# etemesi254/zune-jpeg

Hardware: NVIDIA B200
Metric: decoded MP/s (dequant+IDCT+upsample+YCbCr→RGB), 4K 4:2:0 batch @1/2/4/8 B200 (higher is better)
Workload: dtype int32

## Files before the change

### zune-jpeg_b200/csrc/zj_capi.cu

```cuda
#include <cuda_runtime.h>
#include <stdint.h>
#include <stdio.h>
#include <stdlib.h>
#include <string.h>

#include <algorithm>
#include <atomic>
#include <chrono>
#include <functional>
#include <mutex>
#include <new>
#include <thread>
#include <vector>

#include "../../include/zune_jpeg_b200.h"
#include "zj_device.h"

namespace zj {
cudaError_t launch_group(const DevImage *d_images, const LaunchGroup &g, cudaStream_t stream);
cudaError_t launch_convert(const ConvImage *d_images, uint32_t count, uint32_t nc, uint32_t max_ow, uint32_t max_oh, const zj_output_desc &d, cudaStream_t s);
cudaError_t launch_resize(const ResizeImage *d_images, uint32_t count, uint32_t nc, const zj_output_desc &d, const zj_resize &r, cudaStream_t s);
}

using namespace zj;
// ... 96 lines not shown
    d.mcu_x = mcu_x; d.n_strips = n_strips;
    d.Wp = img->comp[0].width_stride;
    d.W = img->n_comp == 3 ? img->comp[1].width_stride : 0;
    d.stride = w * (uint32_t)nc;
    d.T = 0xffffffffu;
    d.small_width = 0;
    d.hv_avx = (mode == MODE_HV && img->variant == ZJ_VARIANT_X86 && (size_t)16 * d.W >= 500) ? 1u : 0u;
    for (uint32_t z = 0; z < img->n_comp; z++)
        for (int k = 0; k < 32; k++)
            d.qtw[z][k] = (uint32_t)img->comp[z].qt[2 * k] | ((uint32_t)img->comp[z].qt[2 * k + 1] << 24);

    if (kind == OUT_GRAY) {
        const size_t len = (size_t)rows * d.Wp;
        if (n_strips > 0 && len / w != rows) return ZJ_ERR_REF_PANIC;
        d.gray_rows_ok = 1;
        d.gray_brows = n_strips * (rows / 8);
        pl->fast = img->variant == ZJ_VARIANT_X86 && !getenv("ZJ_NO_FAST");
        if (pl->fast) {
            const uint32_t ucols = (d.Wp + 15) / 16;
            d.n_tiles = (ucols + ZF_XU_GRAY - 1) / ZF_XU_GRAY;
            d.tile_q = ucols / d.n_tiles;
            d.tile_r = ucols % d.n_tiles;
            pl->grid_strips = (d.gray_brows + 1) / 2;
        } else {
            d.n_tiles = (d.Wp / 8 + ZJ_THREADS - 1) / ZJ_THREADS;
        }
        pl->grid_tiles = d.n_tiles;
    } else if (kind == OUT_YCC) {
        d.n_norm = w; d.P = 3 * w;
    } else if (kind == OUT_RGB) {
        if (w < 16) {
            if (d.Wp > 16) return ZJ_ERR_REF_PANIC;
            d.small_width = 1;
        } else {
            const uint32_t E = d.Wp / 16 > 0 ? d.Wp / 16 - 1 : 0;
            d.n_norm = 16 * E;
            d.P = 48 * E;
            if (d.P > d.stride) return ZJ_ERR_REF_PANIC;
            const uint32_t room = d.stride - d.P;
            const uint32_t diff = room < 64 ? 64 - room : 0;
            d.T = d.P > diff ? d.P - diff : 0;
            if (d.T + 48 > d.stride) return ZJ_ERR_REF_PANIC;
        }
    }
    if (kind != OUT_GRAY) {
        pl->fast = img->variant == ZJ_VARIANT_X86 && (kind == OUT_RGB || kind == OUT_YCC) && !d.small_width && (d.stride & 3u) == 0 &&
                   (mode != MODE_HV || d.hv_avx) && (reinterpret_cast<uintptr_t>(out) & 3) == 0 && !getenv("ZJ_NO_FAST");
        if (pl->fast) {
            const uint32_t xuv[4] = {ZF_XU_NONE, ZF_XU_H, ZF_XU_V, ZF_XU_HV};
            const uint32_t ucols = (d.Wp + 15) / 16;
            d.n_tiles = (ucols + xuv[mode] - 1) / xuv[mode];
            d.tile_q = ucols / d.n_tiles;
            d.tile_r = ucols % d.n_tiles;
        } else {
            const int tmv[4] = {TM_NONE, TM_H, TM_V, TM_HV};
            d.n_tiles = (mcu_x + tmv[mode] - 1) / tmv[mode];
            d.tile_q = mcu_x / d.n_tiles;
            d.tile_r = mcu_x % d.n_tiles;
        }
        pl->grid_tiles = d.n_tiles;
        d.magic_w = d.W ? (((uint64_t)1 << 40) + d.W - 1) / d.W : 0;
    }
    return ZJ_OK;
}

static int check_buffers(const zj_image *img, const Plan &pl, const void *out, size_t out_len)
{
    for (uint32_t z = 0; z < pl.ncomp_used; z++) {
        if (!img->comp[z].coeff) return ZJ_ERR_INVALID_ARG;
        if (img->comp[z].n_i16 < (uint64_t)pl.n_strips * pl.chunk[z]) return ZJ_ERR_SHORT_PLANE;
    }
    if (!out) return ZJ_ERR_INVALID_ARG;
    if (out_len < pl.out_size) return ZJ_ERR_SHORT_OUTPUT;
    return ZJ_OK;
}

static int check_device_alignment(const zj_image *img, const Plan &pl)
{
    for (uint32_t z = 0; z < pl.ncomp_used; z++)
        if (reinterpret_cast<uintptr_t>(img->comp[z].coeff) & 15) return ZJ_ERR_INVALID_ARG;
    return ZJ_OK;
}

struct zj_batch {
    int device;
    std::vector<LaunchGroup> groups;
    std::vector<std::pair<uint8_t *, size_t>> zero_only;
    DevImage *d_images;
    size_t n_images;
    uint64_t algo_bytes;
    cudaStream_t pool_stream;
    bool pooled;
};

static cudaMemPool_t g_pool[64] = {};
static std::mutex g_pool_mu;
static cudaMemPool_t device_pool(int device)
{
    if (device < 0 || device >= 64) return nullptr;
    std::lock_guard<std::mutex> lock(g_pool_mu);
    if (!g_pool[device]) {
        cudaMemPoolProps props = {};
        props.allocType = cudaMemAllocationTypePinned;
        props.handleTypes = cudaMemHandleTypeNone;
        props.location.type = cudaMemLocationTypeDevice;
        props.location.id = device;
// ... 996 lines not shown
```

### zune-jpeg_b200/csrc/zj_kernels.cu

```cuda
#include <cuda_runtime.h>
#include <stdint.h>
#include <stdlib.h>

#include <type_traits>

#include "zj_device.h"

#define ZF_LIKELY(x) __builtin_expect(!!(x), 1)
#define ZF_UNLIKELY(x) __builtin_expect(!!(x), 0)

namespace zj {

typedef uint32_t u32;

template <int K> __device__ __forceinline__ u32 madk(u32 a, u32 c) { u32 d; asm("mad.lo.s32 %0, %1, %2, %3;" : "=r"(d) : "r"(a), "n"(K), "r"(c)); return d; }

template <int SH>
__device__ __forceinline__ void idct8(u32 &s0, u32 &s1, u32 &s2, u32 &s3, u32 &s4, u32 &s5, u32 &s6, u32 &s7, const u32 bias)
{
    const u32 p1 = (s2 + s6) * 2217u;
    const u32 t2 = madk<-7567>(s6, p1), t3 = madk<3135>(s2, p1);
    const u32 v = (s0 << 12) + bias;
    const u32 t0 = madk<4096>(s4, v), t1 = madk<-4096>(s4, v);
    const u32 x0 = t0 + t3, x3 = t0 - t3, x1 = t1 + t2, x2 = t1 - t2;
// ... 968 lines not shown
    u32 w[12];
#pragma unroll
    for (int k = 0; k < 4; k++) {
        const u32 yE = evens(yw[k]), yO = odds(yw[k]);
        u32 c0E, c1E, c2E, c0O, c1O, c2O;
        if (ycc) {
            c0E = yE; c1E = cbE[k]; c2E = crE[k]; c0O = yO; c1O = cbO[k]; c2O = crO[k];
        } else {
            convert_pair_hi(yE, cbE[k], crE[k], c0E, c1E, c2E, kk, kr);
            convert_pair_hi(yO, cbO[k], crO[k], c0O, c1O, c2O, kk, kr);
        }
        const u32 rgE = prmt(c0E, c1E, sel);
        const u32 brO = prmt(c2E, c0O, sel);
        const u32 gbO = prmt(c1O, c2O, sel);
        w[3 * k] = prmt(rgE, brO, 0x5410u);
        w[3 * k + 1] = prmt(gbO, rgE, 0x7610u);
        w[3 * k + 2] = prmt(brO, gbO, 0x7632u);
    }
    if (ZF_LIKELY(vec && nw == 12)) {
        uint4 *d = reinterpret_cast<uint4 *>(dst);
        d[0] = make_uint4(w[0], w[1], w[2], w[3]); d[1] = make_uint4(w[4], w[5], w[6], w[7]); d[2] = make_uint4(w[8], w[9], w[10], w[11]);
    } else if (vec && nw == 8) {
        uint4 *d = reinterpret_cast<uint4 *>(dst);
        d[0] = make_uint4(w[0], w[1], w[2], w[3]); d[1] = make_uint4(w[4], w[5], w[6], w[7]);
    } else {
        u32 *d = reinterpret_cast<u32 *>(dst);
#pragma unroll
        for (int k = 0; k < 12; k++) if (k < nw) d[k] = w[k];
    }
}

__device__ __forceinline__ void load16(const uint8_t *p, const bool a16, u32 w[4])
{
    if (a16) { const uint4 v = *reinterpret_cast<const uint4 *>(p); w[0] = v.x; w[1] = v.y; w[2] = v.z; w[3] = v.w; }
    else { const uint2 v0 = *reinterpret_cast<const uint2 *>(p), v1 = *reinterpret_cast<const uint2 *>(p + 8); w[0] = v0.x; w[1] = v0.y; w[2] = v1.x; w[3] = v1.y; }
}

constexpr int ZF_NB = 2;
enum { BAR_FULL = 1, BAR_EMPTY = 3, BAR_QUEUE = 5 };

template <int MODE>
__global__ void __launch_bounds__(ZF_THREADS, ZF_MINBLOCKS)
reconstruct_fast_kernel(const DevImage *__restrict__ images, const int spc)
{
    typedef FastTraits<MODE> FT;
    typedef uint8_t ST;
    constexpr int ROWS = FT::ROWS, TWY = FT::TWY, CS = FT::CS, NRG = FT::NRG, XU = FT::XU, RPU = FT::RPU;
    constexpr bool HALO = FT::NSLOT > 0;

    extern __shared__ __align__(128) uint8_t sDynAll[];
    ST *const sPlanes = sDynAll + 3 * ZF_PRODUCERS * 128 + 128;
    __shared__ __align__(16) u32 sQ[3][32];
    __shared__ int sSlowN;
    __shared__ unsigned short sSlow[ZJ_SLOW_CAP];

    const DevImage &im = images[blockIdx.z];
    const u32 tile = blockIdx.x;
    if (tile >= im.n_tiles) return;
    const int tid = threadIdx.x;
    const u32 stride = im.stride;
    uint8_t *__restrict__ out = im.out;
    const u32 n_strips = im.n_strips;
    const u32 s_begin = blockIdx.y * (u32)spc;

    if (s_begin >= n_strips) {
        if (s_begin >= n_strips + (u32)spc) return;
        const size_t lo = (size_t)n_strips * ROWS * stride, hi = (size_t)im.height * stride;
        if (lo >= hi) return;
        const size_t span = hi - lo, per = (span + im.n_tiles - 1) / im.n_tiles;
        size_t b0 = lo + (size_t)tile * per, b1 = b0 + per;
        if (b1 > hi) b1 = hi;
        for (size_t b = b0 + tid; b < b1; b += ZF_THREADS) out[b] = 0;
        return;
    }
    const int n_it = (int)(min(s_begin + (u32)spc, n_strips) - s_begin);

    const int nt = (int)im.n_tiles;
    const int u0 = (int)(tile * im.tile_q + min(tile, im.tile_r)), u1 = (int)((tile + 1) * im.tile_q + min(tile + 1, im.tile_r));
    const int Wp = (int)im.Wp, W = (int)im.W, mcu_x = (int)im.mcu_x;
    const int X0 = 16 * u0;
    const int yb0 = 2 * u0, nyb = min(2 * u1, Wp >> 3) - yb0;
    const int cb0 = FT::H == 2 ? u0 : yb0, ncb = FT::H == 2 ? u1 - u0 : nyb;
    const int lhb = HALO ? (cb0 == 0 ? mcu_x - 1 : cb0 - 1) : -1;
    const int rhb = HALO ? (cb0 + ncb == mcu_x ? 0 : cb0 + ncb) : -1;
    const int spb = (MODE == MODE_HV && tile == 0 && nt > 1) ? mcu_x - 2 : -1;
    const u32 n_norm = im.n_norm, T = im.T, P = im.P;

    for (int k = tid; k < 96; k += ZF_THREADS) sQ[k >> 5][k & 31] = im.qtw[k >> 5][k & 31];
    if (tid == 0) sSlowN = 0;
    __syncthreads();

    const bool producer = tid < ZF_PRODUCERS;
    const int rtid = producer ? tid : tid - ZF_PRODUCERS;
    if (producer) {
        constexpr int NHB = FT::NSLOT * FT::CBR;
        const int lane = tid & 31, wq = ((rtid >> 5) + (int)(blockIdx.x + blockIdx.y + blockIdx.z)) & 3;
        const int ybpr = Wp >> 3;
        auto decode = [&](int b, int &comp, int &br, int &gcol, int &lcol) {
            if (b < FT::NY) { comp = 0; br = b / FT::YB; const int bc = b % FT::YB; gcol = bc < nyb ? yb0 + bc : -1; lcol = bc * 8; }
            else if (b < FT::NY + 2 * FT::NC) {
                int c = b - FT::NY; comp = 1 + c / FT::NC; c %= FT::NC;
                br = c / FT::CB; const int bc = c % FT::CB; gcol = bc < ncb ? cb0 + bc : -1; lcol = 8 + bc * 8;
            } else {
                int hx = b - FT::NY - 2 * FT::NC; comp = 1 + hx / (NHB > 0 ? NHB : 1); hx %= (NHB > 0 ? NHB : 1);
                const int slot = hx / FT::CBR; br = hx % FT::CBR;
                gcol = slot == 0 ? lhb : (slot == 1 ? rhb : spb);
                lcol = slot == 0 ? 0 : (slot == 1 ? 8 + ncb * 8 : 16 + ncb * 8);
                if (NHB == 0 || comp > 2) { comp = 1; gcol = -1; }
            }
        };
        auto block_ptr = [&](int comp, int br, int gcol) -> const int16_t * {
            return comp == 0 ? im.coeff[0] + (((size_t)s_begin * FT::YBR + br) * ybpr + gcol) * 64
                             : im.coeff[comp] + (((size_t)s_begin * FT::CBR + br) * mcu_x + gcol) * 64;
        };
        const u32 stepY = (u32)(FT::YBR * ybpr * 64), stepC = (u32)(FT::CBR * mcu_x * 64);
        auto setup_job = [&](const int B0, u32 &pkj, const int16_t *&g0, const int16_t *&g1, u32 &jmj) {
            int comp, br, gcol, lcol;
            decode(B0 + lane, comp, br, gcol, lcol);
            const bool active = gcol >= 0;
            pkj = (comp == 0 ? (u32)(br * 8 * TWY + lcol) : (u32)(FT::YBYTES + (comp - 1) * FT::CBYTES + br * 8 * CS + lcol)) |
                  (active ? 0x10000u : 0u) | (comp ? 0x20000u : 0u) | ((u32)comp << 18) |
                  ((comp != 0 && lcol == 0) ? 0x100000u : 0u);
            const int lsub = lane >> 3, lch = lane & 7;
            g0 = g1 = im.coeff[0];
            int mode = 0, lim0 = 0, lim1 = 0;
            if (FT::DENSE) {
                if (active) { mode = 3; g0 = block_ptr(comp, br, gcol); }
            } else if (B0 < FT::NY + 2 * FT::NC) {
                int c0, b0r, gg0, l0;
                decode(B0, c0, b0r, gg0, l0);
                const bool isY = B0 < FT::NY;
                const int bpr = isY ? FT::YB : FT::CB;
                const int col0 = isY ? (B0 % FT::YB) : ((B0 - FT::NY) % FT::NC) % FT::CB;
                const int have = (isY ? nyb : ncb) - col0;
                const int first = (isY ? yb0 : cb0) + col0;
                if (bpr >= 32) { mode = 1; lim0 = min(max(have, 0), 32) - lsub; g0 = block_ptr(c0, b0r, first) + lsub * 64 + lch * 8; }
                else {
                    mode = 2; lim0 = lim1 = min(max(have, 0), 16) - lsub;
                    g0 = block_ptr(c0, b0r, first) + lsub * 64 + lch * 8;
                    g1 = block_ptr(c0, b0r + 1, first) + lsub * 64 + lch * 8;
                }
            } else if (active) { mode = 3; g0 = block_ptr(comp, br, gcol); }
            u32 m = 0;
            for (int k = 0; k < 8; k++) {
                const bool second = mode == 2 && k >= 4;
                if ((mode == 1 || mode == 2) && 4 * (second ? k - 4 : k) < (second ? lim1 : lim0)) m |= 1u << k;
            }
            if (mode == 3) m = 0x100u;
            if (mode == 2) g1 -= 4 * 256;
            else g1 = g0;
            jmj = m;
        };
        const u32 stage0 = (u32)__cvta_generic_to_shared(sDynAll) + (u32)(wq * 32) * 128u;
        const u32 d_even = stage0 + (u32)(lane >> 3) * 128u + (u32)(((lane & 7) ^ (lane >> 3)) * 16);
        const u32 d_odd = stage0 + (u32)(lane >> 3) * 128u + (u32)(((lane & 7) ^ ((lane >> 3) + 4)) * 16);
        const u32 slx = (stage0 + (u32)lane * 128u) | (u32)((lane & 7) * 16);
        const u32 scr = (u32)__cvta_generic_to_shared(sDynAll) + ZF_PRODUCERS * 128u + (u32)rtid * 16u;
        const u32 zslot = ((u32)__cvta_generic_to_shared(sDynAll) + 3u * ZF_PRODUCERS * 128u) | (u32)((lane & 7) * 16);
        if (rtid < 8) sts128(zslot - (u32)((lane & 7) * 16) + (u32)rtid * 16u, 0u, 0u, 0u, 0u);
        asm volatile("bar.sync %0, %1;" ::"r"((int)BAR_QUEUE + 1), "n"(ZF_PRODUCERS) : "memory");
        asm volatile("" : "+r"(const_cast<u32 &>(d_even)), "+r"(const_cast<u32 &>(d_odd)), "+r"(const_cast<u32 &>(slx)), "+r"(const_cast<u32 &>(scr)));
        auto issue = [&](const int16_t *g0, const int16_t *g1, const u32 m) {
            if (ZF_LIKELY(m == 0xffu)) {
#pragma unroll
                for (int k = 0; k < 8; k++)
                    asm volatile("cp.async.cg.shared.global [%0], [%1], 16;" ::"r"(((k & 1) ? d_odd : d_even) + k * 512u), "l"((k < 4 ? g0 : g1) + k * 256) : "memory");
            } else if (m & 0x100u) {
#pragma unroll
                for (int r = 0; r < 8; r++)
                    asm volatile("cp.async.cg.shared.global [%0], [%1], 16;" ::"r"(slx ^ (u32)(r << 4)), "l"(g0 + r * 8) : "memory");
            } else {
#pragma unroll
                for (int k = 0; k < 8; k++)
                    if (m & (1u << k))
                        asm volatile("cp.async.cg.shared.global [%0], [%1], 16;" ::"r"(((k & 1) ? d_odd : d_even) + k * 512u), "l"((k < 4 ? g0 : g1) + k * 256) : "memory");
            }
            asm volatile("cp.async.commit_group;" ::: "memory");
        };
        u32 pk[2], jm[2];
        const int16_t *q0[2], *q1[2];
#pragma unroll
        for (int ps = 0; ps < 2; ps++) {
            const int jw = ps == 0 ? wq : ((wq + ((MODE == MODE_NONE || MODE == MODE_H) ? 2 : 0)) & 3);
            setup_job(ps * ZF_PRODUCERS + jw * 32, pk[ps], q0[ps], q1[ps], jm[ps]);
        }
        const int16_t *qa0 = q0[0], *qb0 = q1[0], *qa1 = q0[1], *qb1 = q1[1];
        const u32 pk0 = pk[0], pk1 = pk[1], jm0 = jm[0], jm1 = jm[1];
        const u32 st0 = FT::DENSE ? ((pk0 & 0x20000u) ? stepC : stepY) : ((wq * 32 < FT::NY) ? stepY : stepC);
        const u32 st1 = FT::DENSE ? ((pk1 & 0x20000u) ? stepC : stepY) : ((ZF_PRODUCERS + wq * 32 < FT::NY) ? stepY : stepC);
        const bool work0 = __any_sync(0xffffffffu, (pk0 & 0x10000u) != 0), work1 = __any_sync(0xffffffffu, (pk1 & 0x10000u) != 0);
        issue(qa0, qb0, jm0);
        qa0 += st0; qb0 += st0;
        int buf = 0;
        for (int it = 0; it < n_it; it++) {
            ST *planes = sPlanes + buf * FT::BUF;
#pragma unroll 1
            for (int ps = 0; ps < 2; ps++) {
                if (ps == 1 && !work1) break;
                const u32 pkk = ps ? pk1 : pk0;
                const bool active = (pkk & 0x10000u) != 0;
                asm volatile("cp.async.wait_group 0;" ::: "memory");
                __syncwarp();
                if (ps == 0 && it >= ZF_NB) bar_sync(BAR_EMPTY + buf);
                auto refill = [&]() {
                    const bool nxt = ps || !work1;
                    issue(nxt ? qa0 : qa1, nxt ? qb0 : qb1, nxt ? (it + 1 < n_it ? jm0 : 0u) : jm1);
                    if (nxt) { qa0 += st0; qb0 += st0; } else { qa1 += st1; qb1 += st1; }
                };
                if (ps ? work1 : work0) idct_rolled<FT::IDCT_UNROLL, FT::LO6>(active, active ? slx : zslot, scr, sQ[(pkk >> 18) & 3u], planes + (pkk & 0xffffu), (pkk & 0x20000u) ? CS : TWY, refill);
                else refill();
            }
            bar_arrive(BAR_FULL + buf);
            buf = buf + 1 == ZF_NB ? 0 : buf + 1;
        }
        return;
    }

    const int tc = rtid;
    const int xu = tc % XU, rgA = tc / XU;
    const bool ycc = im.out_kind == OUT_YCC;
    u32 esel = !ycc ? 0x7351u : 0x6240u, ekk = 0xC000C000u ^ ((u32)spc >> 30);
    asm volatile("" : "+r"(esel), "+r"(ekk));
    u32 ekr = 0x98619861u ^ ((u32)spc >> 30);
    asm volatile("" : "+r"(ekr));
    int xs = X0 + 16 * xu;
    int kind = 0;
    int dst_off = 3 * xs, nw = 12;
    if (u0 + xu < u1 && rgA < NRG / 2) {
        if ((u32)(xs + 16) <= n_norm) {
            kind = 1;
            if (T != 0xffffffffu && (u32)(3 * xs + 48) > T && (u32)(3 * xs) < T + 48) {
                const int keep = (int)T - 3 * xs;
                if ((u32)(3 * xs + 48) > T + 48) kind = 2;
                else if (keep <= 0) kind = 0;
                else if ((keep & 3) == 0) nw = keep >> 2;
                else kind = 2;
            }
        } else if (T != 0xffffffffu && (u0 + xu) == ((Wp - 16) >> 4)) {
            kind = 1; xs = Wp - 16; dst_off = (int)T;
        } else if ((u32)xs < n_norm) {
            kind = 2;
        }
    }
    if (kind == 1 && (dst_off & 3) != 0) kind = 2;
    const bool vec = ((stride & 15u) == 0) && ((reinterpret_cast<uintptr_t>(out) & 15) == 0) && ((dst_off & 15) == 0) && ((nw & 3) == 0);
    const int xl = xs - X0;
    const bool y16 = (xl & 15) == 0;
    const int cc0 = FT::H == 2 ? xs >> 1 : xs;
    const int lc = 8 + (cc0 - cb0 * 8);
    const bool first_x = HALO && cc0 == 0, last_x = HALO && cc0 + 8 == W;
    int kindA = kind, kindB = kind;
    int off0 = 0, off2 = 0;
    bool sel0 = false, firstvec = false, hv_tail = false;
    const int pbit = rgA & 1;
    if (MODE == MODE_H) {
        off0 = first_x ? -CS : 0; off2 = last_x ? CS : 0;
    } else if (MODE == MODE_HV) {
        off0 = (first_x && pbit) ? -CS : 0; off2 = last_x ? CS : 0;
        sel0 = (((pbit ? W : 0) + cc0) & 15) == 0;
        firstvec = pbit == 0 && cc0 < 16;
        hv_tail = pbit == 1 && cc0 + 16 >= W;
        if (kind == 1 && hv_tail && W - 36 - cb0 * 8 < (cb0 == 0 ? 0 : -8)) kindA = kindB = 2;
        if (kind == 1 && firstvec && W < 48) kindA = kindB = 2;
    }
#pragma unroll
    for (int h = 0; h < 2; h++)
        if ((h ? kindB : kindA) == 2) {
            const int slot = atomicAdd(&sSlowN, 1);
            if (slot < ZJ_SLOW_CAP) sSlow[slot] = (unsigned short)(((rgA + h * (NRG / 2)) << 8) | (xl >> 3));
        }
    bar_sync_consumers(BAR_QUEUE);
    const int nslow = sSlowN;

    const u32 z0 = (T != 0xffffffffu && T + 48 > P) ? T + 48 : P;
    const u32 zlen = stride > z0 ? stride - z0 : 0;
    const int zg = (((z0 | stride) & 15u) == 0 && (reinterpret_cast<uintptr_t>(out) & 15) == 0) ? 16 : ((((z0 | stride) & 3u) == 0 && (reinterpret_cast<uintptr_t>(out) & 3) == 0) ? 4 : 1);
    const u32 zper = ((zlen / zg + nt - 1) / nt) * zg;
    const u32 zb0 = min(z0 + tile * zper, stride), zb1 = min(zb0 + zper, stride);
    const int zcnt = (int)((zb1 - zb0) / zg);
    const int zrpp = (zcnt > 0 && zcnt < ZF_CONSUMERS) ? ZF_CONSUMERS / zcnt : 1;
    const int zr0 = (zcnt > 0 && zcnt < ZF_CONSUMERS) ? (tc / zcnt < zrpp ? tc / zcnt : ROWS) : 0;
    const int zk0 = (zcnt > 0 && zcnt < ZF_CONSUMERS) ? tc % zcnt : tc;

    int buf = 0;
    for (int it = 0; it < n_it; it++) {
        const ST *planes = sPlanes + buf * FT::BUF;
        const u32 y_base = (s_begin + it) * ROWS;
        bar_sync(BAR_FULL + buf);
#pragma unroll 1
        for (int h = 0; h < 2; h++) {
            if ((h ? kindB : kindA) != 1) continue;
            const int rg = rgA + h * (NRG / 2);
            int yl0, yl1, ra, rb;
            if (MODE == MODE_V) { yl0 = 2 * rg; yl1 = yl0 + 1; ra = rg; rb = (rg == 0 || rg == 7) ? rg : rg + 1; }
            else if (MODE == MODE_HV) { const int j = rg >> 1; yl0 = 4 * j + pbit; yl1 = yl0 + 2; ra = 2 * j + pbit; rb = (j == 0 || j == 7) ? ra : ra + 2; }
            else { yl0 = rg; yl1 = rg; ra = rg; rb = rg; }
            u32 E0[2][4], O0[2][4], E1[2][4], O1[2][4];
#pragma unroll
            for (int c = 0; c < 2; c++) {
                const uint8_t *base = planes + FT::YBYTES + c * FT::CBYTES;
                if (MODE == MODE_NONE) {
                    u32 w[4];
                    load16(base + ra * CS + lc, false, w);
#pragma unroll
                    for (int k = 0; k < 4; k++) { E0[c][k] = evens(w[k]); O0[c][k] = odds(w[k]); }
                } else if (MODE == MODE_V) {
                    u32 a[4], b[4];
                    load16(base + ra * CS + lc, false, a);
                    load16(base + rb * CS + lc, false, b);
#pragma unroll
                    for (int k = 0; k < 4; k++) {
                        const u32 aE = evens(a[k]), aO = odds(a[k]), bE = evens(b[k]), bO = odds(b[k]);
                        T2pair(aE, bE, E0[c][k], E1[c][k]);
                        T2pair(aO, bO, O0[c][k], O1[c][k]);
                    }
                } else if (MODE == MODE_H) {
                    const uint8_t *pa = base + ra * CS + lc;
                    const uint2 a = *reinterpret_cast<const uint2 *>(pa);
                    const bool hstart = first_x && rg == 0, hend = last_x && rg == NRG - 1;
                    const u32 left = hstart ? (a.x & 0xffu) : (u32)pa[off0 - 1], right = hend ? 0u : (u32)pa[off2 + 8];
                    const u32 r[4] = {lanes01(a.x), lanes23(a.x), lanes01(a.y), lanes23(a.y)};
                    hfilter16(left | (right << 16), r, E0[c], O0[c]);
                    if (ZF_UNLIKELY(hend)) {
                        const u32 e3 = E0[c][3], o3 = O0[c][3];
                        O0[c][2] = prmt(O0[c][2], r[2], 0x7610u);
                        E0[c][3] = prmt(r[3], o3, 0x5410u);
                        O0[c][3] = prmt(e3, r[3], 0x7610u);
                    }
                } else if (ZF_LIKELY(!hv_tail)) {
                    const uint8_t *pa = base + ra * CS + lc, *pb = base + rb * CS + lc;
                    const uint2 a = *reinterpret_cast<const uint2 *>(pa), b = *reinterpret_cast<const uint2 *>(pb);
                    const u32 aL = pa[off0 - 1], aR = pa[off2 + 8], bL = pb[off0 - 1], bR = pb[off2 + 8];
                    const u32 A[4] = {lanes01(a.x), lanes23(a.x), lanes01(a.y), lanes23(a.y)};
                    const u32 B[4] = {lanes01(b.x), lanes23(b.x), lanes01(b.y), lanes23(b.y)};
                    const u32 Ah = aL | (aR << 16), Bh = bL | (bR << 16);
                    u32 N[4], F[4];
                    u32 Nh, Fh;
#pragma unroll
                    for (int k = 0; k < 4; k++) T2pair_s(A[k], B[k], N[k], F[k]);
                    T2pair_s(Ah, Bh, Nh, Fh);
                    u32 pv = (3u * ((sel0 ? (a.x & 0xffu) + (b.x & 0xffu) : aR + bR) + 2u)) >> 2;
                    if (ZF_UNLIKELY(firstvec)) {
                        const int j = rg >> 1;
                        if (j == 0) pv = sel0 ? (a.x & 0xffu) : aR;
                        else if (sel0) {
                            const int spc0 = nt > 1 ? 16 + ncb * 8 : 8 + (W - 16);
                            const int rp = 2 * j - 1, rq = (j == 1) ? rp : rp + 2;
                            pv = (3u * ((u32)base[rp * CS + spc0] + (u32)base[rq * CS + spc0] + 2u)) >> 2;
                        } else {
                            const u32 y0 = base[2 * j * CS + 8], y1 = (j == 1) ? y0 : (j == 7 ? 0u : (u32)base[(2 * j + 2) * CS + 8]);
                            pv = (3u * (y0 + y1 + 2u)) >> 2;
                        }
                    }
                    pv = pv * 4u;
                    const u32 keep = sel0 ? 0xffff0000u : 0x0000ffffu, ins = sel0 ? pv : pv << 16;
                    Nh = (Nh & keep) | ins;
                    Fh = (Fh & keep) | ins;
                    hfilter16_s(Nh, N, E0[c], O0[c]);
                    hfilter16_s(Fh, F, E1[c], O1[c]);
                    if (firstvec && cc0 == 0) E1[c][0] = prmt(E1[c][0], O1[c][0], 0x3254u);
                } else {
                    const int q = (cc0 - (W - 16)) >> 3;
                    const int lq = 8 + (W - 36 + 8 * q - cb0 * 8);
#pragma unroll
                    for (int f = 0; f < 2; f++) {
                        const u32 *pw = reinterpret_cast<const u32 *>(base + (f ? rb : ra) * CS + lq);
                        const u32 w0 = pw[0], w1 = pw[1], w2 = pw[2];
                        const u32 r[4] = {prmt(w0, w1, 0x0403u) & 0x00ff00ffu, prmt(w1, 0u, 0x4241u), prmt(w1, w2, 0x0403u) & 0x00ff00ffu, prmt(w2, 0u, 0x4241u)};
                        const u32 hh = prmt(w0, w2, 0x0702u) & 0x00ff00ffu;
                        u32 *E = f ? E1[c] : E0[c], *O = f ? O1[c] : O0[c];
                        hfilter16(hh, r, E, O);
                        if (q == 1) { E[3] = prmt(E[3], 0u, 0x1010u); O[3] = prmt(O[3], 0u, 0x1010u); }
                    }
                }
            }
            if (y_base + yl0 < im.height) {
                u32 yw[4];
                load16(planes + yl0 * TWY + xl, FT::H == 2 || y16, yw);
                emit16(out + (size_t)(y_base + yl0) * stride + dst_off, yw, E0[0], O0[0], E0[1], O0[1], ycc, nw, vec, esel, ekk, ekr);
            }
            if (RPU == 2 && y_base + yl1 < im.height) {
                u32 yw[4];
                load16(planes + yl1 * TWY + xl, FT::H == 2 || y16, yw);
                emit16(out + (size_t)(y_base + yl1) * stride + dst_off, yw, E1[0], O1[0], E1[1], O1[1], ycc, nw, vec, esel, ekk, ekr);
            }
        }
        if (ZF_UNLIKELY(nslow > 0)) {
            SlowCtx<ST> sc;
#pragma unroll
            for (int c = 0; c < 2; c++) {
                sc.cv[c].base = planes + FT::YBYTES + c * FT::CBYTES; sc.cv[c].W = W; sc.cv[c].n = FT::CROWS * W;
                sc.cv[c].c0 = cb0 * 8; sc.cv[c].c1 = (cb0 + ncb) * 8; sc.cv[c].lhb = lhb; sc.cv[c].rhb = rhb; sc.cv[c].spb = spb; sc.cv[c].cs = CS; sc.cv[c].magic_w = im.magic_w;
            }
            sc.sY = planes; sc.twy = TWY; sc.X0 = X0; sc.Wp = Wp; sc.hv_avx = (int)im.hv_avx; sc.y_base = y_base; sc.height = im.height;
            sc.stride = stride; sc.n_norm = n_norm; sc.T = T; sc.ycc = ycc; sc.out = out; sc.width = im.width; sc.nc = im.nc;
            if (nslow > ZJ_SLOW_CAP) {
                const int tw = nyb * 8;
                for (int u0s = 0; u0s < ROWS * tw; u0s += ZF_CONSUMERS) {
                    const int u = u0s + tc;
                    if (u < ROWS * tw) { const int yl = u / tw; slow_pixel<MODE, 0, ST>(sc, yl, u - yl * tw); }
                }
            } else {
                const int total = nslow * 16 * RPU;
                for (int t0s = 0; t0s < total; t0s += ZF_CONSUMERS) {
                    const int t = t0s + tc;
                    if (t < total) {
                        const int e = sSlow[t / (16 * RPU)], r = (t >> 4) % RPU, k = t & 15;
                        const int g = e >> 8, xl2 = (e & 0xff) << 3;
                        int yl;
                        if (MODE == MODE_V) yl = 2 * g + r;
                        else if (MODE == MODE_HV) yl = 4 * (g >> 1) + (g & 1) + 2 * r;
                        else yl = g;
                        if (xl2 + k < nyb * 8) slow_pixel<MODE, 0, ST>(sc, yl, xl2 + k);
                    }
                }
            }
            __syncwarp();
        }
        if (it + ZF_NB < n_it) bar_arrive(BAR_EMPTY + buf);
        buf = buf + 1 == ZF_NB ? 0 : buf + 1;
        if (ZF_UNLIKELY(zcnt > 0)) {
            for (int yl = zr0; yl < ROWS; yl += zrpp) {
                const u32 y = y_base + (u32)yl;
                if (y >= im.height) break;
                uint8_t *zrow = out + (size_t)y * stride + zb0;
                for (int k = zk0; k < zcnt; k += ZF_CONSUMERS) {
                    uint8_t *z = zrow + (size_t)k * zg;
                    if (zg == 16) *reinterpret_cast<uint4 *>(z) = make_uint4(0u, 0u, 0u, 0u);
                    else if (zg == 4) *reinterpret_cast<u32 *>(z) = 0u;
                    else *z = 0;
                }
            }
            __syncwarp();
        }
    }
}

template <int VARIANT>
__global__ void __launch_bounds__(ZJ_THREADS)
gray_kernel(const DevImage *__restrict__ images, int rows_per_strip)
{
    typedef typename std::conditional<VARIANT == 0, uint8_t, int16_t>::type ST;
    __shared__ __align__(16) ST sT[ZJ_THREADS][64 + 8];
    __shared__ u32 sQ[32];
    const DevImage &im = images[blockIdx.z];
    const int tid = threadIdx.x;
    const int ybpr = (int)(im.Wp >> 3);
    const u32 brows = im.n_strips * (u32)(rows_per_strip >> 3);
    const u32 br = blockIdx.y;
    uint8_t *__restrict__ out = im.out;
    if (br >= brows) {
        if (br > brows) return;
        const size_t lo = (size_t)brows * 8 * im.stride, hi = (size_t)im.height * im.stride;
        if (lo >= hi) return;
        const size_t span = hi - lo, per = (span + gridDim.x - 1) / gridDim.x;
        size_t b0 = lo + (size_t)blockIdx.x * per, b1 = b0 + per;
        if (b1 > hi) b1 = hi;
        for (size_t b = b0 + tid; b < b1; b += ZJ_THREADS) out[b] = 0;
        return;
    }
    if (tid < 32) sQ[tid] = im.qtw[0][tid];
    __syncthreads();
    const int bc = blockIdx.x * ZJ_THREADS + tid;
    const bool active = bc < ybpr;
    const size_t blk = (size_t)br * ybpr + (active ? bc : 0);
    int4 raw[8];
    load_block(active, im.coeff[0] + blk * 64, raw);
    idct_block<VARIANT, ST>(active, raw, sQ, &sT[tid][0], 8);
    if (!active) return;
    const u32 x0 = (u32)bc * 8;
#pragma unroll 1
    for (int r = 0; r < 8; r++) {
        const u32 y = br * 8 + r;
        if (y >= im.height) break;
        uint8_t *row = out + (size_t)y * im.stride;
        for (int k = 0; k < 8; k++)
            if (x0 + k < im.width) row[x0 + k] = (uint8_t)((u32)sT[tid][r * 8 + k] & 0xff);
    }
}

template <int MODE, int VARIANT>
static cudaError_t launch_reconstruct(const DevImage *d_images, const LaunchGroup &g, cudaStream_t stream)
{
    dim3 grid(g.max_tiles, g.max_strips + 1, g.count);
    reconstruct_kernel<MODE, VARIANT><<<grid, ZJ_THREADS, 0, stream>>>(d_images + g.first);
    return cudaGetLastError();
}
// ... 75 lines not shown
            else refill();
            bar_arrive(BAR_FULL + (it & 1));
        }
        return;
    }

    const int tc = tid - ZF_PRODUCERS;
    const int xu = tc & 31, rgA = tc >> 5;
    const int xs = X0 + 16 * xu, xl = 16 * xu;
    const int npx = (u0 + xu < u1) ? min(max((int)width - xs, 0), 16) : 0;
    const bool vec = npx == 16 && (stride & 15u) == 0 && (reinterpret_cast<uintptr_t>(out) & 15) == 0;
    const bool words = npx == 16 && (stride & 3u) == 0 && (reinterpret_cast<uintptr_t>(out) & 3) == 0;
    for (int it = 0; it < n_it; it++) {
        const uint8_t *planes = sPlanes + (it & 1) * ZG_BUF;
        const u32 y_base = (s_begin + (u32)it) * ZG_ROWS;
        bar_sync(BAR_FULL + (it & 1));
        if (npx > 0) {
#pragma unroll
            for (int h = 0; h < 4; h++) {
                const int rg = rgA + 4 * h;
                const u32 y = y_base + (u32)rg;
                if (y >= height) continue;
                uint4 v = make_uint4(0u, 0u, 0u, 0u);
                if (y < brows * 8u) v = *reinterpret_cast<const uint4 *>(planes + rg * ZG_TW + xl);
                uint8_t *d = out + (size_t)y * stride + xs;
                if (vec) *reinterpret_cast<uint4 *>(d) = v;
                else if (words) { u32 *dw = reinterpret_cast<u32 *>(d); dw[0] = v.x; dw[1] = v.y; dw[2] = v.z; dw[3] = v.w; }
                else {
                    const u32 w[4] = {v.x, v.y, v.z, v.w};
#pragma unroll
                    for (int k = 0; k < 16; k++) if (k < npx) d[k] = (uint8_t)(w[k >> 2] >> (8 * (k & 3)));
                }
            }
        }
        if (it + 2 < n_it) bar_arrive(BAR_EMPTY + (it & 1));
    }
}

static int strips_per_cta(const LaunchGroup &g)
{
    static int forced = -1, slots = 0;
    if (forced < 0) {
        const char *e = getenv("ZJ_SPC");
        forced = e ? (atoi(e) < 1 ? 1 : atoi(e)) : 0;
    }
    if (forced) return forced;
    if (slots == 0) {
        int dev = 0, sms = 0;
        cudaGetDevice(&dev);
        if (cudaDeviceGetAttribute(&sms, cudaDevAttrMultiProcessorCount, dev) != cudaSuccess || sms <= 0) sms = 148;
        slots = 3 * sms;
    }
    const long S = g.max_strips > 0 ? (long)g.max_strips : 1;
    long parts = (S + ZF_DEFAULT_SPC - 1) / ZF_DEFAULT_SPC;
    const long columns = (long)g.max_tiles * (long)g.count;
    while (columns * parts < 2L * slots && S / parts > 4) parts++;
    return (int)((S + parts - 1) / parts);
}

template <int MODE>
static cudaError_t launch_fast(const DevImage *d_images, const LaunchGroup &g, cudaStream_t stream)
{
    const int spc = strips_per_cta(g);
    dim3 grid(g.max_tiles, (g.max_strips + spc - 1) / spc + 1, g.count);
    typedef FastTraits<MODE> FT;
    constexpr size_t smem = 3 * ZF_PRODUCERS * 128 + 128 + (size_t)ZF_NB * FT::BUF;
    static bool configured[64] = {false};
    int dev = 0;
    cudaGetDevice(&dev);
    if (dev >= 0 && dev < 64 && !configured[dev]) {
        cudaError_t e = cudaFuncSetAttribute(reconstruct_fast_kernel<MODE>, cudaFuncAttributeMaxDynamicSharedMemorySize, (int)smem);
        if (e != cudaSuccess) return e;
        configured[dev] = true;
    }
    reconstruct_fast_kernel<MODE><<<grid, ZF_THREADS, smem, stream>>>(d_images + g.first, spc);
    return cudaGetLastError();
}

static cudaError_t launch_gray_fast(const DevImage *d_images, const LaunchGroup &g, cudaStream_t stream)
{
    const int spc = strips_per_cta(g);
    dim3 grid(g.max_tiles, (g.max_strips + spc - 1) / spc + 1, g.count);
    constexpr size_t smem = 3 * ZF_PRODUCERS * 128 + 128 + 2 * ZG_BUF;
    static bool configured[64] = {false};
    int dev = 0;
    cudaGetDevice(&dev);
    if (dev >= 0 && dev < 64 && !configured[dev]) {
        cudaError_t e = cudaFuncSetAttribute(gray_fast_kernel, cudaFuncAttributeMaxDynamicSharedMemorySize, (int)smem);
        if (e != cudaSuccess) return e;
        configured[dev] = true;
    }
    gray_fast_kernel<<<grid, ZF_THREADS, smem, stream>>>(d_images + g.first, spc);
    return cudaGetLastError();
}

cudaError_t launch_group(const DevImage *d_images, const LaunchGroup &g, cudaStream_t stream)
{
    if (g.gray && g.fast) return launch_gray_fast(d_images, g, stream);
    if (g.fast) {
        switch (g.mode) {
        case MODE_NONE: return launch_fast<MODE_NONE>(d_images, g, stream);
        case MODE_H: return launch_fast<MODE_H>(d_images, g, stream);
        case MODE_V: return launch_fast<MODE_V>(d_images, g, stream);
        default: return launch_fast<MODE_HV>(d_images, g, stream);
        }
    }
    if (g.gray) {
        const int rows = g.mode == MODE_NONE ? 8 : (g.mode == MODE_HV ? 32 : 16);
        dim3 grid(g.max_tiles, g.max_strips * (rows >> 3) + 1, g.count);
        if (g.variant == 0) gray_kernel<0><<<grid, ZJ_THREADS, 0, stream>>>(d_images + g.first, rows);
        else gray_kernel<1><<<grid, ZJ_THREADS, 0, stream>>>(d_images + g.first, rows);
        return cudaGetLastError();
    }
    switch (g.mode * 2 + g.variant) {
    case MODE_NONE * 2 + 0: return launch_reconstruct<MODE_NONE, 0>(d_images, g, stream);
    case MODE_NONE * 2 + 1: return launch_reconstruct<MODE_NONE, 1>(d_images, g, stream);
    case MODE_H * 2 + 0: return launch_reconstruct<MODE_H, 0>(d_images, g, stream);
// ... 10 lines not shown
```

Baseline: 642,000.

## Walk all HV tiles within one CTA per strip band, reusing chroma halo columns

For 4:2:0 (HV) output, the grid now launches a single CTA column per strip band. Each CTA walks every horizontal tile of each strip in sequence, with the producer/consumer pipeline running over tile×strip steps. The right chroma halo of the previous tile is copied from the other shared-memory buffer, so producers skip reloading those blocks. Interior tiles take a precomputed fast geometry path that bypasses the slow queue setup. The cost is more sequential work per CTA and less grid parallelism across tile columns, which strips_per_cta tries to offset by splitting strips more finely.

```diff
diff --git a/zune-jpeg_b200/csrc/zj_capi.cu b/zune-jpeg_b200/csrc/zj_capi.cu
--- a/zune-jpeg_b200/csrc/zj_capi.cu
+++ b/zune-jpeg_b200/csrc/zj_capi.cu
@@ -172,6 +172,10 @@
             d.n_tiles = (ucols + xuv[mode] - 1) / xuv[mode];
             d.tile_q = ucols / d.n_tiles;
             d.tile_r = ucols % d.n_tiles;
+            if (mode == MODE_HV) {
+                d.tile_q = std::min(ucols, (uint32_t)ZF_XU_HV);
+                d.tile_r = 0;
+            }
         } else {
             const int tmv[4] = {TM_NONE, TM_H, TM_V, TM_HV};
             d.n_tiles = (mcu_x + tmv[mode] - 1) / tmv[mode];
diff --git a/zune-jpeg_b200/csrc/zj_kernels.cu b/zune-jpeg_b200/csrc/zj_kernels.cu
--- a/zune-jpeg_b200/csrc/zj_kernels.cu
+++ b/zune-jpeg_b200/csrc/zj_kernels.cu
@@ -1044,6 +1044,7 @@
     ST *const sPlanes = sDynAll + 3 * ZF_PRODUCERS * 128 + 128;
     __shared__ __align__(16) u32 sQ[3][32];
     __shared__ int sSlowN;
+    __shared__ int sEdge;
     __shared__ unsigned short sSlow[ZJ_SLOW_CAP];
 
     const DevImage &im = images[blockIdx.z];
@@ -1059,7 +1060,8 @@
         if (s_begin >= n_strips + (u32)spc) return;
         const size_t lo = (size_t)n_strips * ROWS * stride, hi = (size_t)im.height * stride;
         if (lo >= hi) return;
-        const size_t span = hi - lo, per = (span + im.n_tiles - 1) / im.n_tiles;
+        const u32 nzt = MODE == MODE_HV ? 1u : im.n_tiles;
+        const size_t span = hi - lo, per = (span + nzt - 1) / nzt;
         size_t b0 = lo + (size_t)tile * per, b1 = b0 + per;
         if (b1 > hi) b1 = hi;
         for (size_t b = b0 + tid; b < b1; b += ZF_THREADS) out[b] = 0;
@@ -1079,7 +1081,7 @@
     const u32 n_norm = im.n_norm, T = im.T, P = im.P;
 
     for (int k = tid; k < 96; k += ZF_THREADS) sQ[k >> 5][k & 31] = im.qtw[k >> 5][k & 31];
-    if (tid == 0) sSlowN = 0;
+    if (tid == 0) { sSlowN = 0; if (MODE == MODE_HV) sEdge = max(((((int)Wp + 15) >> 4) - 4) / XU, 1); }
     __syncthreads();
 
     const bool producer = tid < ZF_PRODUCERS;
@@ -1111,8 +1113,7 @@
             decode(B0 + lane, comp, br, gcol, lcol);
             const bool active = gcol >= 0;
             pkj = (comp == 0 ? (u32)(br * 8 * TWY + lcol) : (u32)(FT::YBYTES + (comp - 1) * FT::CBYTES + br * 8 * CS + lcol)) |
-                  (active ? 0x10000u : 0u) | (comp ? 0x20000u : 0u) | ((u32)comp << 18) |
-                  ((comp != 0 && lcol == 0) ? 0x100000u : 0u);
+                  (active ? 0x10000u : 0u) | (comp ? 0x20000u : 0u) | ((u32)comp << 18);
             const int lsub = lane >> 3, lch = lane & 7;
             g0 = g1 = im.coeff[0];
             int mode = 0, lim0 = 0, lim1 = 0;
@@ -1175,6 +1176,60 @@
         for (int ps = 0; ps < 2; ps++) {
             const int jw = ps == 0 ? wq : ((wq + ((MODE == MODE_NONE || MODE == MODE_H) ? 2 : 0)) & 3);
             setup_job(ps * ZF_PRODUCERS + jw * 32, pk[ps], q0[ps], q1[ps], jm[ps]);
+        }
+        if (MODE == MODE_HV) {
+            const int ucols = (Wp + 15) >> 4, wlast = max(ucols - XU, 0);
+            const int jw1 = wq;
+            const int16_t *const ybase = q0[0], *const cbase = q0[1];
+            const ptrdiff_t drun = q1[1] - q0[1];
+            const u32 pky = pk[0], pkc = pk[1], jmy = jm[0], jmc = jm[1];
+            const bool worky = __any_sync(0xffffffffu, (pky & 0x10000u) != 0);
+            const int n_steps = n_it * nt;
+            issue(ybase, ybase, jmy);
+            int t = 0, s = 0, buf = 0;
+            for (int st = 0; st < n_steps; st++) {
+                ST *planes = sPlanes + buf * FT::BUF;
+                const bool first = t == 0, last = t == nt - 1;
+                int tn = t + 1, sn = s;
+                if (tn == nt) { tn = 0; sn++; }
+                const int16_t *const qn = ybase + (size_t)sn * stepY + (tn == nt - 1 ? wlast : XU * tn) * 128;
+                const int16_t *qa1 = cbase + (size_t)s * stepC + (last ? wlast : XU * t + 1) * 64, *qb1 = qa1 + drun;
+                u32 pk1 = pkc + (last ? 0u : 8u), jm1 = jmc;
+                const bool work1 = jw1 < 2 || (jw1 == 2 && (first || last));
+                if (jw1 == 2 && work1) {
+                    const int comp = lane < 6 ? 1 : 2, hx = lane < 6 ? lane : lane - 6, slot = hx >> 1, br = hx & 1;
+                    int gcol, lcol;
+                    if (last) { gcol = slot == 0 ? (wlast == 0 ? mcu_x - 1 : wlast - 1) : (slot == 1 ? 0 : -1); lcol = slot == 0 ? 0 : 8 + 8 * (ucols - wlast); }
+                    else { gcol = slot == 0 ? mcu_x - 1 : (slot == 1 ? 0 : mcu_x - 2); lcol = slot == 0 ? 0 : (slot == 1 ? 8 : 16 + FT::TWC); }
+                    const bool act = lane < 12 && gcol >= 0;
+                    pk1 = (u32)(FT::YBYTES + (comp - 1) * FT::CBYTES + br * 8 * CS + lcol) | (act ? 0x10000u : 0u) | 0x20000u | ((u32)comp << 18);
+                    qa1 = qb1 = im.coeff[comp] + (((size_t)(s_begin + s) * FT::CBR + br) * mcu_x + (act ? gcol : 0)) * 64;
+                    jm1 = act ? 0x100u : 0u;
+                }
+#pragma unroll 1
+                for (int ps = 0; ps < 2; ps++) {
+                    if (ps == 1 && !work1) break;
+                    const u32 pkk = ps ? pk1 : pky;
+                    const bool active = (pkk & 0x10000u) != 0;
+                    asm volatile("cp.async.wait_group 0;" ::: "memory");
+                    __syncwarp();
+                    if (ps == 0 && st >= ZF_NB) bar_sync(BAR_EMPTY + buf);
+                    if (ps == 1 && jw1 < 2 && !first && !last) {
+                        const u32 o = (u32)(FT::YBYTES + jw1 * FT::CBYTES + (lane >> 1) * CS + (lane & 1) * 8);
+                        *reinterpret_cast<uint2 *>(planes + o) = *reinterpret_cast<const uint2 *>(sPlanes + (buf ^ 1) * FT::BUF + o + FT::TWC);
+                    }
+                    auto refill = [&]() {
+                        const bool nxt = ps || !work1;
+                        issue(nxt ? qn : qa1, nxt ? qn : qb1, nxt ? (st + 1 < n_steps ? jmy : 0u) : jm1);
+                    };
+                    if (ps ? work1 : worky) idct_rolled<FT::IDCT_UNROLL, FT::LO6>(active, active ? slx : zslot, scr, sQ[(pkk >> 18) & 3u], planes + (pkk & 0xffffu), (pkk & 0x20000u) ? CS : TWY, refill);
+                    else refill();
+                }
+                bar_arrive(BAR_FULL + buf);
+                buf = buf + 1 == ZF_NB ? 0 : buf + 1;
+                t = tn; s = sn;
+            }
+            return;
         }
         const int16_t *qa0 = q0[0], *qb0 = q1[0], *qa1 = q0[1], *qb1 = q1[1];
         const u32 pk0 = pk[0], pk1 = pk[1], jm0 = jm[0], jm1 = jm[1];
@@ -1215,10 +1270,28 @@
     asm volatile("" : "+r"(esel), "+r"(ekk));
     u32 ekr = 0x98619861u ^ ((u32)spc >> 30);
     asm volatile("" : "+r"(ekr));
-    int xs = X0 + 16 * xu;
-    int kind = 0;
-    int dst_off = 3 * xs, nw = 12;
-    if (u0 + xu < u1 && rgA < NRG / 2) {
+    struct TileGeom { int u0, u1, e0, X0, cb0, ncb, nyb, lhb, rhb, spb; };
+    const int ucols = (Wp + 15) >> 4;
+    auto tile_geom = [&](const int t) {
+        TileGeom g;
+        if (MODE == MODE_HV) {
+            g.e0 = XU * t; g.u1 = min(g.e0 + XU, ucols); g.u0 = t == nt - 1 ? max(ucols - XU, 0) : g.e0;
+            g.X0 = 16 * g.u0; g.cb0 = g.u0; g.ncb = g.u1 - g.u0; g.nyb = min(2 * g.u1, Wp >> 3) - 2 * g.u0;
+            g.lhb = g.cb0 == 0 ? mcu_x - 1 : g.cb0 - 1; g.rhb = g.cb0 + g.ncb == mcu_x ? 0 : g.cb0 + g.ncb; g.spb = (t == 0 && nt > 1) ? mcu_x - 2 : -1;
+        } else {
+            g.u0 = u0; g.u1 = u1; g.e0 = u0; g.X0 = X0; g.cb0 = cb0; g.ncb = ncb; g.nyb = nyb; g.lhb = lhb; g.rhb = rhb; g.spb = spb;
+        }
+        return g;
+    };
+    int xs, kind, dst_off, nw, xl, cc0, lc, kindA, kindB, off0, off2;
+    bool vec, y16, first_x, last_x, sel0, firstvec, hv_tail;
+    const int pbit = rgA & 1;
+    auto unit_setup = [&](const TileGeom &g) {
+    const int cu0 = g.u0, cu1 = g.u1, ce0 = g.e0, cX0 = g.X0, ccb0 = g.cb0;
+    xs = cX0 + 16 * xu;
+    kind = 0;
+    dst_off = 3 * xs; nw = 12;
+    if ((MODE != MODE_HV || cu0 + xu >= ce0) && cu0 + xu < cu1 && rgA < NRG / 2) {
         if ((u32)(xs + 16) <= n_norm) {
             kind = 1;
             if (T != 0xffffffffu && (u32)(3 * xs + 48) > T && (u32)(3 * xs) < T + 48) {
@@ -1228,23 +1301,22 @@
                 else if ((keep & 3) == 0) nw = keep >> 2;
                 else kind = 2;
             }
-        } else if (T != 0xffffffffu && (u0 + xu) == ((Wp - 16) >> 4)) {
+        } else if (T != 0xffffffffu && (cu0 + xu) == ((Wp - 16) >> 4)) {
             kind = 1; xs = Wp - 16; dst_off = (int)T;
         } else if ((u32)xs < n_norm) {
             kind = 2;
         }
     }
     if (kind == 1 && (dst_off & 3) != 0) kind = 2;
-    const bool vec = ((stride & 15u) == 0) && ((reinterpret_cast<uintptr_t>(out) & 15) == 0) && ((dst_off & 15) == 0) && ((nw & 3) == 0);
-    const int xl = xs - X0;
-    const bool y16 = (xl & 15) == 0;
-    const int cc0 = FT::H == 2 ? xs >> 1 : xs;
-    const int lc = 8 + (cc0 - cb0 * 8);
-    const bool first_x = HALO && cc0 == 0, last_x = HALO && cc0 + 8 == W;
-    int kindA = kind, kindB = kind;
-    int off0 = 0, off2 = 0;
-    bool sel0 = false, firstvec = false, hv_tail = false;
-    const int pbit = rgA & 1;
+    vec = ((stride & 15u) == 0) && ((reinterpret_cast<uintptr_t>(out) & 15) == 0) && ((dst_off & 15) == 0) && ((nw & 3) == 0);
+    xl = xs - cX0;
+    y16 = (xl & 15) == 0;
+    cc0 = FT::H == 2 ? xs >> 1 : xs;
+    lc = 8 + (cc0 - ccb0 * 8);
+    first_x = HALO && cc0 == 0; last_x = HALO && cc0 + 8 == W;
+    kindA = kind; kindB = kind;
+    off0 = 0; off2 = 0;
+    sel0 = false; firstvec = false; hv_tail = false;
     if (MODE == MODE_H) {
         off0 = first_x ? -CS : 0; off2 = last_x ? CS : 0;
     } else if (MODE == MODE_HV) {
@@ -1252,33 +1324,55 @@
         sel0 = (((pbit ? W : 0) + cc0) & 15) == 0;
         firstvec = pbit == 0 && cc0 < 16;
         hv_tail = pbit == 1 && cc0 + 16 >= W;
-        if (kind == 1 && hv_tail && W - 36 - cb0 * 8 < (cb0 == 0 ? 0 : -8)) kindA = kindB = 2;
+        if (kind == 1 && hv_tail && W - 36 - ccb0 * 8 < (ccb0 == 0 ? 0 : -8)) kindA = kindB = 2;
         if (kind == 1 && firstvec && W < 48) kindA = kindB = 2;
     }
+    };
+    int qbase = 0, nslow = 0;
+    auto queue_slow = [&]() {
 #pragma unroll
     for (int h = 0; h < 2; h++)
         if ((h ? kindB : kindA) == 2) {
-            const int slot = atomicAdd(&sSlowN, 1);
+            const int slot = atomicAdd(&sSlowN, 1) - qbase;
             if (slot < ZJ_SLOW_CAP) sSlow[slot] = (unsigned short)(((rgA + h * (NRG / 2)) << 8) | (xl >> 3));
         }
     bar_sync_consumers(BAR_QUEUE);
-    const int nslow = sSlowN;
+    const int qend = sSlowN;
+    nslow = qend - qbase;
+    qbase = qend;
+    };
+    if (MODE != MODE_HV) { unit_setup(tile_geom(0)); queue_slow(); }
 
     const u32 z0 = (T != 0xffffffffu && T + 48 > P) ? T + 48 : P;
     const u32 zlen = stride > z0 ? stride - z0 : 0;
     const int zg = (((z0 | stride) & 15u) == 0 && (reinterpret_cast<uintptr_t>(out) & 15) == 0) ? 16 : ((((z0 | stride) & 3u) == 0 && (reinterpret_cast<uintptr_t>(out) & 3) == 0) ? 4 : 1);
-    const u32 zper = ((zlen / zg + nt - 1) / nt) * zg;
+    const u32 zper = MODE == MODE_HV ? zlen : ((zlen / zg + nt - 1) / nt) * zg;
     const u32 zb0 = min(z0 + tile * zper, stride), zb1 = min(zb0 + zper, stride);
     const int zcnt = (int)((zb1 - zb0) / zg);
     const int zrpp = (zcnt > 0 && zcnt < ZF_CONSUMERS) ? ZF_CONSUMERS / zcnt : 1;
     const int zr0 = (zcnt > 0 && zcnt < ZF_CONSUMERS) ? (tc / zcnt < zrpp ? tc / zcnt : ROWS) : 0;
     const int zk0 = (zcnt > 0 && zcnt < ZF_CONSUMERS) ? tc % zcnt : tc;
+    const u32 zpk = (u32)zr0 | ((u32)zrpp << 8) | ((u32)zk0 << 16);
 
     int buf = 0;
-    for (int it = 0; it < n_it; it++) {
+    const int it_end = MODE == MODE_HV ? 0 : n_it;
+    int tcol = 0;
+    u32 yrow = s_begin * ROWS;
+    for (int it = MODE == MODE_HV ? -n_it * nt : 0; it < it_end; it++) {
         const ST *planes = sPlanes + buf * FT::BUF;
-        const u32 y_base = (s_begin + it) * ROWS;
+        const u32 y_base = MODE == MODE_HV ? yrow : (s_begin + it) * ROWS;
         bar_sync(BAR_FULL + buf);
+        if (MODE == MODE_HV) {
+            if ((u32)(tcol - 1) >= (u32)(sEdge - 1)) {
+                unit_setup(tile_geom(tcol));
+                queue_slow();
+            } else {
+                xs = 16 * (XU * tcol + xu); dst_off = 3 * xs; nw = 12; xl = 16 * xu; lc = 8 + 8 * xu;
+                vec = ((stride & 15u) == 0) && ((reinterpret_cast<uintptr_t>(out) & 15) == 0);
+                sel0 = (((pbit ? W : 0) + 8 * xu) & 15) == 0;
+                kindA = kindB = 1; off0 = off2 = 0; firstvec = hv_tail = false; nslow = 0;
+            }
+        }
 #pragma unroll 1
         for (int h = 0; h < 2; h++) {
             if ((h ? kindB : kindA) != 1) continue;
@@ -1336,7 +1430,7 @@
                         const int j = rg >> 1;
                         if (j == 0) pv = sel0 ? (a.x & 0xffu) : aR;
                         else if (sel0) {
-                            const int spc0 = nt > 1 ? 16 + ncb * 8 : 8 + (W - 16);
+                            const int spc0 = nt > 1 ? 16 + FT::CB * 8 : 8 + (W - 16);
                             const int rp = 2 * j - 1, rq = (j == 1) ? rp : rp + 2;
                             pv = (3u * ((u32)base[rp * CS + spc0] + (u32)base[rq * CS + spc0] + 2u)) >> 2;
                         } else {
@@ -1353,7 +1447,7 @@
                     if (firstvec && cc0 == 0) E1[c][0] = prmt(E1[c][0], O1[c][0], 0x3254u);
                 } else {
                     const int q = (cc0 - (W - 16)) >> 3;
-                    const int lq = 8 + (W - 36 + 8 * q - cb0 * 8);
+                    const int lq = 8 + (W - 36 + 8 * q - (MODE == MODE_HV ? tile_geom(tcol).cb0 : cb0) * 8);
 #pragma unroll
                     for (int f = 0; f < 2; f++) {
                         const u32 *pw = reinterpret_cast<const u32 *>(base + (f ? rb : ra) * CS + lq);
@@ -1378,16 +1472,17 @@
             }
         }
         if (ZF_UNLIKELY(nslow > 0)) {
+            const TileGeom tg = tile_geom(MODE == MODE_HV ? tcol : 0);
             SlowCtx<ST> sc;
 #pragma unroll
             for (int c = 0; c < 2; c++) {
                 sc.cv[c].base = planes + FT::YBYTES + c * FT::CBYTES; sc.cv[c].W = W; sc.cv[c].n = FT::CROWS * W;
-                sc.cv[c].c0 = cb0 * 8; sc.cv[c].c1 = (cb0 + ncb) * 8; sc.cv[c].lhb = lhb; sc.cv[c].rhb = rhb; sc.cv[c].spb = spb; sc.cv[c].cs = CS; sc.cv[c].magic_w = im.magic_w;
-            }
-            sc.sY = planes; sc.twy = TWY; sc.X0 = X0; sc.Wp = Wp; sc.hv_avx = (int)im.hv_avx; sc.y_base = y_base; sc.height = im.height;
+                sc.cv[c].c0 = tg.cb0 * 8; sc.cv[c].c1 = (tg.cb0 + tg.ncb) * 8; sc.cv[c].lhb = tg.lhb; sc.cv[c].rhb = tg.rhb; sc.cv[c].spb = tg.spb; sc.cv[c].cs = CS; sc.cv[c].magic_w = im.magic_w;
+            }
+            sc.sY = planes; sc.twy = TWY; sc.X0 = tg.X0; sc.Wp = Wp; sc.hv_avx = (int)im.hv_avx; sc.y_base = y_base; sc.height = im.height;
             sc.stride = stride; sc.n_norm = n_norm; sc.T = T; sc.ycc = ycc; sc.out = out; sc.width = im.width; sc.nc = im.nc;
             if (nslow > ZJ_SLOW_CAP) {
-                const int tw = nyb * 8;
+                const int tw = tg.nyb * 8;
                 for (int u0s = 0; u0s < ROWS * tw; u0s += ZF_CONSUMERS) {
                     const int u = u0s + tc;
                     if (u < ROWS * tw) { const int yl = u / tw; slow_pixel<MODE, 0, ST>(sc, yl, u - yl * tw); }
@@ -1403,20 +1498,25 @@
                         if (MODE == MODE_V) yl = 2 * g + r;
                         else if (MODE == MODE_HV) yl = 4 * (g >> 1) + (g & 1) + 2 * r;
                         else yl = g;
-                        if (xl2 + k < nyb * 8) slow_pixel<MODE, 0, ST>(sc, yl, xl2 + k);
+                        if (xl2 + k < tg.nyb * 8) slow_pixel<MODE, 0, ST>(sc, yl, xl2 + k);
                     }
                 }
             }
             __syncwarp();
         }
-        if (it + ZF_NB < n_it) bar_arrive(BAR_EMPTY + buf);
+        if (it + ZF_NB < it_end) bar_arrive(BAR_EMPTY + buf);
         buf = buf + 1 == ZF_NB ? 0 : buf + 1;
         if (ZF_UNLIKELY(zcnt > 0)) {
-            for (int yl = zr0; yl < ROWS; yl += zrpp) {
-                const u32 y = y_base + (u32)yl;
+            const int zt = MODE == MODE_HV ? tcol : 0, zn = MODE == MODE_HV ? nt : 1;
+            u32 zp = zpk;
+            if (MODE == MODE_HV) asm volatile("" : "+r"(zp));
+            const int zr = MODE == MODE_HV ? (int)(zp & 0xffu) : zr0, zs = MODE == MODE_HV ? (int)((zp >> 8) & 0xffu) : zrpp;
+            const int zk = MODE == MODE_HV ? (int)(zp >> 16) : zk0;
+            for (int j = zr; zt + j * zn < ROWS; j += zs) {
+                const u32 y = y_base + (u32)(zt + j * zn);
                 if (y >= im.height) break;
                 uint8_t *zrow = out + (size_t)y * stride + zb0;
-                for (int k = zk0; k < zcnt; k += ZF_CONSUMERS) {
+                for (int k = zk; k < zcnt; k += ZF_CONSUMERS) {
                     uint8_t *z = zrow + (size_t)k * zg;
                     if (zg == 16) *reinterpret_cast<uint4 *>(z) = make_uint4(0u, 0u, 0u, 0u);
                     else if (zg == 4) *reinterpret_cast<u32 *>(z) = 0u;
@@ -1425,6 +1525,7 @@
             }
             __syncwarp();
         }
+        if (MODE == MODE_HV && ++tcol == nt) { tcol = 0; yrow += ROWS; }
     }
 }
 
@@ -1606,9 +1707,12 @@
         slots = 3 * sms;
     }
     const long S = g.max_strips > 0 ? (long)g.max_strips : 1;
-    long parts = (S + ZF_DEFAULT_SPC - 1) / ZF_DEFAULT_SPC;
-    const long columns = (long)g.max_tiles * (long)g.count;
-    while (columns * parts < 2L * slots && S / parts > 4) parts++;
+    const bool walk = !g.gray && g.mode == MODE_HV;
+    const long steps = walk ? (long)g.max_tiles : 1;
+    long parts = (S * steps + ZF_DEFAULT_SPC - 1) / ZF_DEFAULT_SPC;
+    if (parts > S) parts = S;
+    const long columns = (walk ? 1L : (long)g.max_tiles) * (long)g.count;
+    while (columns * parts < 2L * slots && (S / parts) * steps > 4 && parts < S) parts++;
     return (int)((S + parts - 1) / parts);
 }
 
@@ -1616,7 +1720,7 @@
 static cudaError_t launch_fast(const DevImage *d_images, const LaunchGroup &g, cudaStream_t stream)
 {
     const int spc = strips_per_cta(g);
-    dim3 grid(g.max_tiles, (g.max_strips + spc - 1) / spc + 1, g.count);
+    dim3 grid(MODE == MODE_HV ? 1 : g.max_tiles, (g.max_strips + spc - 1) / spc + 1, g.count);
     typedef FastTraits<MODE> FT;
     constexpr size_t smem = 3 * ZF_PRODUCERS * 128 + 128 + (size_t)ZF_NB * FT::BUF;
     static bool configured[64] = {false};
```

After: 552,200 (median of 6 runs). 0.86x the previous value.
